# hucsmn/suffix_array

Hardware: AMD Instinct MI355X
Metric: input MB/s indexed (SA build) (higher is better)
Workload: dtype u8; 1 GPU; c3_english_256m: 268435456 bytes per GPU, seed base + rank, one independent text per GPU; n_bytes=268435456, sigma=57, symbols_per_key=13, refinement_rounds=9, text_rounds=0, radix_passes=25, unresolved_after_initial_sort=199000237

## Files before the change

suffix_array_amd/__init__.py:

```python
from __future__ import annotations

import ctypes
import os
from typing import Optional

import numpy as np

__all__ = ["MAX_LENGTH", "saca", "SuffixArray", "SuffixArrayError", "lib", "diag_lib", "library_path", "Stats", "last_host_timing",
           "saca_batch", "workspace_bytes", "device_pci_bus_id", "saca_device_ptr", "bucket_table", "check_integrity", "last_stats", "DeviceIndex", "pack", "unpack",
           "lcp", "saca_lcp", "last_lcp_stats", "lcp_work_bytes", "lcp_device_ptr", "LcpStats",
           "lcp_set_compare_cap", "last_search_stats", "SearchStats",
           "bwt", "unbwt", "bwt_device_ptr", "unbwt_device_ptr", "bwt_work_bytes", "unbwt_work_bytes", "last_unbwt_stats",
           "unbwt_set_walk_limits", "unbwt_set_splitter_spacing", "UnbwtStats",
           "repeat_lengths", "repeat_spans", "last_repeat_stats", "repeats_work_bytes", "repeat_spans_bound",
           "repeat_lengths_device_ptr", "repeat_spans_device_ptr", "RepeatStats", "REPEATS_ALL", "REPEATS_KEEP_FIRST",
           "lpf", "lz77", "lz77_decode", "lz77_literals", "last_lz_stats", "lz_work_bytes", "lpf_device_ptr", "lz77_device_ptr", "LzStats", "LZ_LITERAL",
           "repeated_substrings", "last_substr_stats", "substrings_work_bytes", "substrings_bound", "substrings_device_ptr", "SubstrQuery", "SubstrStats",
           "SUBSTR_ALL", "SUBSTR_BY_COUNT", "SUBSTR_BY_LENGTH", "SUBSTR_BY_COVER",
           "DocSubstrQuery", "DocSubstrStats", "SUBSTR_BY_DOCS", "last_doc_substr_stats", "doc_substrings_work_bytes",
           "MatchStats", "last_match_stats", "match_work_bytes", "match_set_group_cap", "match_set_group_lanes", "match_stats_device_ptr", "match_spans_device_ptr",
           "MATCH_NONE", "MATCH_TILE",
           "DocRepeatStats", "last_doc_repeat_stats", "doc_repeats_work_bytes", "DOCREP_ANY", "DOCREP_OTHER",
           "DocsStats", "last_docs_stats", "docs_set_chunk", "docs_work_bytes", "doc_of_device_ptr", "DOC_NONE", "DOC_SAMPLES",
           "DOC_CHUNK_MIN", "DOC_CHUNK_MAX", "DOC_CHUNK_DEFAULT",
# ... 532 lines not shown
        L.sa_amd_tok_index_next_tokens.argtypes = [c_vp, c_vp, c_vp, ctypes.c_int32, c_vp, c_vp, c_vp, c_vp, c_vp, c_vp, ctypes.c_int64, c_vp]
        L.sa_amd_tok_index_next_tokens.restype = ctypes.c_int32
        L.sa_amd_tok_index_infgram.argtypes = [c_vp, c_vp, c_vp, ctypes.c_int32, ctypes.c_int32, ctypes.c_int32, c_vp, c_vp, c_vp, c_vp, c_vp, c_vp,
                                               c_vp, ctypes.c_int64, c_vp]
        L.sa_amd_tok_index_infgram.restype = ctypes.c_int32
        L.sa_amd_last_tok_stats.argtypes = [c_vp]
        L.sa_amd_last_tok_stats.restype = None
        L.sa_amd_tok_index_infgram_score.argtypes = [c_vp, c_vp, ctypes.c_int64, c_vp, ctypes.c_int64, ctypes.c_int32, ctypes.c_int32, c_vp, c_vp,
                                                     c_vp, c_vp, c_vp, c_vp]
        L.sa_amd_tok_index_infgram_score.restype = ctypes.c_int32
        L.sa_amd_last_tok_score_stats.argtypes = [c_vp]
        L.sa_amd_last_tok_score_stats.restype = None
        for u16_name, u32_name in (("sa_amd_max_tokens_u16", "sa_amd_max_tokens_u32"), ("sa_amd_saca_u16", "sa_amd_saca_u32")) + tuple(
                ("sa_amd_tok_index_" + op, "sa_amd_tok32_index_" + op)
                for op in ("create", "destroy", "sa", "search", "next_tokens", "infgram", "infgram_score")):
            u16_fn, u32_fn = getattr(L, u16_name), getattr(L, u32_name)
            u32_fn.argtypes, u32_fn.restype = u16_fn.argtypes, u16_fn.restype
        _lib = L
    return _lib


_diag: Optional[ctypes.CDLL] = None


def diag_lib() -> ctypes.CDLL:
    global _diag
    if _diag is None:
        path = os.path.join(_HERE, "libsuffix_array_amd_diag.so")
        if not os.path.exists(path):
            raise ImportError(f"{path} not found: run __graft_entry__.build()")
        L = ctypes.CDLL(path)
        c_vp = ctypes.c_void_p
        L.sa_amd_test_sort_pairs.argtypes = [c_vp, c_vp, ctypes.c_int64, ctypes.c_int32, ctypes.c_int32]
        L.sa_amd_test_sort_pairs.restype = ctypes.c_int32
        L.sa_amd_test_sort_pairs32.argtypes = [c_vp, c_vp, ctypes.c_int64, ctypes.c_int32, ctypes.c_int32]
        L.sa_amd_test_sort_pairs32.restype = ctypes.c_int32
        L.sa_amd_test_sort_pairs_flags.argtypes = [c_vp, c_vp, ctypes.c_int64, ctypes.c_int32, ctypes.c_int32, c_vp, c_vp]
        L.sa_amd_test_sort_pairs_flags.restype = ctypes.c_int32
        L.sa_amd_debug_head_flags.argtypes = [ctypes.c_int32]
        L.sa_amd_debug_head_flags.restype = ctypes.c_int32
        L.sa_amd_debug_round_flags.argtypes = [ctypes.c_int32]
        L.sa_amd_debug_round_flags.restype = ctypes.c_int32
        L.sa_amd_debug_fill_blocks.argtypes = [ctypes.c_int32]
        L.sa_amd_debug_fill_blocks.restype = ctypes.c_int32
        L.sa_amd_last_stats.argtypes = [c_vp]
        L.sa_amd_test_sample_sort64.argtypes = [c_vp, c_vp, ctypes.c_int64, ctypes.c_int32, c_vp]
        L.sa_amd_test_sample_sort64.restype = ctypes.c_int32
        L.sa_amd_test_bucket_sort32.argtypes = [c_vp, c_vp, ctypes.c_int64, ctypes.c_int32, c_vp]
        L.sa_amd_test_bucket_sort32.restype = ctypes.c_int32
        L.sa_amd_test_lz_nsv.argtypes = [c_vp, ctypes.c_int64, c_vp, c_vp, c_vp]
        L.sa_amd_test_lz_nsv.restype = ctypes.c_int32
        L.sa_amd_test_build_keys.argtypes = [c_vp, ctypes.c_int32, c_vp, c_vp, c_vp]
        L.sa_amd_test_build_keys.restype = ctypes.c_int32
        L.sa_amd_debug_phase_cycles.argtypes = [c_vp, ctypes.c_int32]
        L.sa_amd_debug_phase_cycles.restype = ctypes.c_int32
        L.sa_amd_debug_group_sort_stamps.argtypes = [ctypes.c_int32]
        L.sa_amd_debug_group_sort_stamps.restype = ctypes.c_int32
        L.sa_amd_debug_rr_count_stamps.argtypes = [ctypes.c_int32]
        L.sa_amd_debug_rr_count_stamps.restype = ctypes.c_int32
        L.sa_amd_debug_sort_variant_count.restype = ctypes.c_int32
        L.sa_amd_debug_sort_variant_name.argtypes = [ctypes.c_int32]
        L.sa_amd_debug_sort_variant_name.restype = ctypes.c_char_p
        L.sa_amd_saca_u8.argtypes = [c_vp, c_vp, ctypes.c_int32]
        L.sa_amd_saca_u8.restype = ctypes.c_int32
        L.sa_amd_saca_device.argtypes = [c_vp, c_vp, ctypes.c_int32, c_vp, ctypes.c_int64, c_vp, c_vp]
        L.sa_amd_saca_device.restype = ctypes.c_int32
        L.sa_amd_workspace_bytes.argtypes = [ctypes.c_int32]
        L.sa_amd_workspace_bytes.restype = ctypes.c_int64
        L.sa_amd_version.restype = ctypes.c_char_p
        _diag = L
    return _diag


def device_pci_bus_id(device: int = 0) -> str:
    buf = ctypes.create_string_buffer(64)
    _check(lib().sa_amd_device_pci_bus_id(int(device), buf, 64))
    return buf.value.decode()


def _check(code: int) -> None:
    if code != 0:
        raise SuffixArrayError(code, lib().sa_amd_strerror(code).decode())


def _as_u8(s) -> np.ndarray:
    if isinstance(s, np.ndarray):
        if s.dtype != np.uint8 or not s.flags.c_contiguous:
            raise TypeError("text must be a contiguous uint8 array")
        return s
    return np.frombuffer(bytes(s), dtype=np.uint8) if len(s) else np.zeros(0, dtype=np.uint8)


def saca(s, sa: np.ndarray) -> None:
    t = _as_u8(s)
    assert t.size <= MAX_LENGTH
    assert t.size + 1 == sa.size
    if sa.dtype != np.uint32 or not sa.flags.c_contiguous or not sa.flags.writeable:
        raise TypeError("sa must be a writable contiguous uint32 array")
    _check(lib().sa_amd_saca_u8(t.ctypes.data, sa.ctypes.data, t.size))


def divsufsort(s, sa: np.ndarray) -> None:
    t = _as_u8(s)
    assert t.size == sa.size and sa.dtype == np.int32
    _check(lib().sa_amd_divsufsort(t.ctypes.data, sa.ctypes.data, t.size))

# ... 1219 lines not shown
```

suffix_array_amd/csrc/host/pipeline.hpp:

```cpp
#pragma once
#include "support.hpp"
#include "tuning.hpp"
#include "pool.hpp"
#include "sort.hpp"
#include "readback.hpp"

#include <functional>

namespace sa {

static inline Tuning env_tuning() { return Tuning::from_env(N_SORT_VARIANTS, N_SORT32_VARIANTS, N_OS_SHAPES64, N_OS_SHAPES32); }
static inline Tuning route_tuning()
{
    const Tuning tn = env_tuning();
    g_posted_off = tn.no_posted_readback;
    return tn;
}

constexpr size_t GRAM_MAX_ENTRIES = (size_t)1 << 24;
static_assert(GROUP_CAP_MAX == GS_CAP, "Tuning clamps SA_AMD_GROUP_CAP to the kernel's cap");

struct Workspace {
    uint64_t *keysA, *keysB, *keysC;
    uint32_t *valsA, *valsB, *isa, *U0, *U1, *G0, *G1;
// ... 101 lines not shown
static int scatter_binned(const SortScratch &ss, uint32_t *isa, uint32_t *pk, uint32_t *pv, uint32_t *altk, uint32_t *altv, int64_t count, int64_t n,
                          hipStream_t st, sa_amd_stats *local, const Tuning &tn, bool iota = false,
                          uint32_t *altk2 = nullptr, uint32_t *altv2 = nullptr)
{
    const int nb = bit_length((uint64_t)(n > 1 ? n : 1));
    int wlog = nb - 16;
    if (wlog < 10) wlog = 10;
    if (wlog > 15) wlog = 15;
    const bool two = nb > wlog && (tn.scatter_levels == 2 || (tn.scatter_levels == 0 && count >= ((int64_t)1 << 25)));
    SortResult<uint32_t> pr;
    if (two) {
        int rc;
        if (iota) {
            const int mid = wlog + RADIX_BITS < nb ? wlog + RADIX_BITS : nb;
            SortJob<uint32_t> first{ pk, nullptr, altk, altv, count, wlog, mid };
            first.iota = true;
            rc = sort_pairs32(first, ss, st, tn, &pr, local);
            if (rc) return rc;
            if (pr.passes != 1) return SA_AMD_EINTERNAL;
            if (mid < nb) {
                rc = sort_pairs32(SortJob<uint32_t>{ altk, altv, altk2, altv2, count, mid, nb }, ss, st, tn, &pr, local);
                if (rc) return rc;
            }
        } else {
            SortJob<uint32_t> both{ pk, pv, altk, altv, count, wlog, nb };
            both.keys_out2 = altk2;
            rc = sort_pairs32(both, ss, st, tn, &pr, local);
            if (rc) return rc;
        }
        const unsigned grid = (unsigned)ceil_div(count, SW_CHUNK);
        if (wlog <= 13)
            PROF(KC_SCATTER, count, st, hipLaunchKernelGGL((k_scatter_windows<13>), dim3(grid), dim3(SW_THREADS), 0, st, (const uint32_t *)pr.keys,
                                                           (const uint32_t *)pr.vals, isa, count, (uint32_t)n, wlog));
        else
            PROF(KC_SCATTER, count, st, hipLaunchKernelGGL((k_scatter_windows<15>), dim3(grid), dim3(SW_THREADS), 0, st, (const uint32_t *)pr.keys,
                                                           (const uint32_t *)pr.vals, isa, count, (uint32_t)n, wlog));
        return SA_AMD_OK;
    }
    const int shift = nb > RADIX_BITS ? nb - RADIX_BITS : 0;
    SortJob<uint32_t> one{ pk, pv, altk, altv, count, shift, shift + RADIX_BITS };
    one.iota = iota;
    const int rc = sort_pairs32(one, ss, st, tn, &pr, local);
    if (rc) return rc;
    PROF(KC_SCATTER, count, st, hipLaunchKernelGGL((k_scatter_pairs<uint32_t>), dim3((unsigned)ceil_div(count, 1024)), dim3(256), 0, st,
                                                   (const uint32_t *)pr.keys, (const uint32_t *)pr.vals, isa, count, (uint32_t)n));
    return SA_AMD_OK;
}

}
#include "refine_round.hpp"
namespace sa {

static int choose_gram_keys(const uint8_t *dT, int64_t n, KeyParams *Pp, int *key_bits, const Workspace &w, hipStream_t st,
                            const Tuning &tn, bool trace)
{
    KeyParams &P = *Pp;
    const uint64_t se = P.sigma;
    const uint64_t cap = (uint64_t)((size_t)n < GRAM_MAX_ENTRIES ? (size_t)n : GRAM_MAX_ENTRIES);
    int g = 0;
    uint64_t S = 1;
    for (int t = 1; t <= 8; ++t) {
        if (S * se > cap) break;
        S *= se; g = t;
        if (tn.gram_g >= 2 && g == tn.gram_g) break;
    }
    if (g < 2) return SA_AMD_OK;
    uint64_t top = 1;
    for (int t = 0; t + 1 < g; ++t) top *= se;
    const int64_t gtiles = ceil_div((int64_t)S, GT_TILE);
    HIP_TRY(hipMemsetAsync(w.gram_flags, 0, (size_t)S, st));
    PROF(KC_MISC, n, st, hipLaunchKernelGGL((k_gram_mark), dim3((unsigned)ceil_div(ceil_div(n, KB_TILE), GM_TPW)), dim3(KB_THREADS), 0, st, dT, n, P, g,
                                            (uint32_t)top, w.gram_flags));
    PROF(KC_MISC, (int64_t)S, st, hipLaunchKernelGGL((k_gram_count), dim3((unsigned)gtiles), dim3(GT_THREADS), 0, st,
                                            (const uint8_t *)w.gram_flags, (int64_t)S, w.tcnt));
    PROF(KC_RR_SCAN, gtiles, st, hipLaunchKernelGGL((k_rr_scan), dim3(1), dim3(SPINE_THREADS), 0, st, w.tcnt, w.thead, gtiles, w.total));
    uint32_t D = 0;
    { const int rcw = read_words(&D, w.total, 4, st); if (rcw) return rcw; }
    int m = 0;
    unsigned __int128 pw = 1;
    while (D >= 2 && (m + 1) * g <= 64 && pw * D <= ((unsigned __int128)1 << 64)) { pw *= D; ++m; }
    int tail = 0;
    while (m > 0 && tail < tn.gram_tail_max && m * g + tail + 1 <= 64 && pw * se <= ((unsigned __int128)1 << 64)) { pw *= se; ++tail; }
    const int gram_bits = m > 0 ? bit_length((uint64_t)(pw - 1)) : 0;
    const int plain_passes = (int)ceil_div(*key_bits, RADIX_BITS), gram_passes = (int)ceil_div(gram_bits, RADIX_BITS);
    const int syms = m * g + tail;
    const bool better = m > 0 && (syms > P.k || (syms == P.k && gram_passes < plain_passes));
    if (trace) fprintf(stderr, "suffix_array_amd: gram keys: %u of %llu %d-grams occur -> %d symbols (%d grams + %d plain) in %d bits (plain: %d in %d) -> %s\n",
                       D, (unsigned long long)S, g, syms, m, tail, gram_bits, P.k, *key_bits, better ? "gram keys" : "plain keys");
    if (!better) return SA_AMD_OK;
    PROF(KC_MISC, (int64_t)S, st, hipLaunchKernelGGL((k_gram_table), dim3((unsigned)gtiles), dim3(GT_THREADS), 0, st,
                                            (const uint8_t *)w.gram_flags, (int64_t)S, (const uint32_t *)w.tcnt, w.gram_table));
    P.gram = g; P.gram_m = m; P.gram_tail = tail; P.gram_top = (uint32_t)top; P.gram_D = D; P.gram_table = w.gram_table;
    P.bits = 0; P.k = syms; P.mask = ~0ull;
    *key_bits = gram_bits;
    return SA_AMD_OK;
}

struct EarlyDownload {
    int off = 0;
    int64_t threshold = 0;
    std::function<void(hipEvent_t)> start;
    std::function<int64_t()> stop;
    bool started = false;
    int64_t m_snap = 0;
    int64_t covered = 0;
    int64_t holes = 0;
    const uint32_t *d_bits = nullptr, *d_tile_off = nullptr, *d_holes = nullptr;
    hipEvent_t ev = nullptr;
};

struct DeviceBuild : BuildCore {
    EarlyDownload *early = nullptr;
    bool trace = false;
    double trace_t = 0;
    double lap() { const double t = now_ms(), d = t - trace_t; trace_t = t; return d; }
    bool timing_only() const
    {
#ifdef SA_AMD_DIAG
        return tn.timing_only_initial_sort;
#else
        return false;
#endif
    }
    KeyParams P, Ptext;
    int sigma = 0, key_bits = 0, top_shift = 0;
    bool force_dense = false, text_ok = false, probe_dense = false;
    SortResult<uint64_t> sr;
    const uint32_t *sorted32 = nullptr;
    int bucket_top_bits = 0;
    bool flat_text = false;
    bool bucket_finished = false;
    uint64_t *sorted0 = nullptr;
    int64_t tiles = 0, depth = 0;
    uint32_t m32 = 0;
    bool lists_ready = false, finished32 = false, fused64 = false, sparse = false;
    bool isa_tail_ranks = false;
    bool tnext_scanned = false;
    int s_sym = 0, tkb = 0;
    bool unary_done = false;
// ... 43 lines not shown
    int choose_bucket_bits() const
    {
        if (tn.no_bucket_sort || n < tn.bucket_min_n || n <= 1) return 0;
        const bool wide_ok = onesweep_on(w.ss, tn) && tn.onesweep32_shape == 0;
        if (tn.bucket_bits == 18 && wide_ok) return 18;
        if (tn.bucket_bits == 16) return 16;
        const bool value_bits = wide_ok && !tn.no_value_bits && !tn.no_text_keys && g_bits <= 30 &&
                                ((sigma == 256 && P.bits == 8) || (sigma == 4 && P.bits == 2 && !tn.no_packed_text));
        if (value_bits && (n >> 16) > 7500 && (n >> 18) * 10 <= bucket_cap_max() * 9) return 18;
        if ((n >> 16) * 10 <= bucket_cap(2) * 9) return 16;
        if (wide_ok && (n >> 18) * 10 <= bucket_cap_max() * 9) return 18;
        if ((n >> 16) * 10 <= bucket_cap_max() * 9) return 16;
        return 0;
    }

    bool flat_rule_applies() const { return n >= 2 && n < tn.top32_probe_min_n && n < ((int64_t)1 << 24) && !tn.no_flat_rule; }

    template <int ISA_MODE>
    int rr_apply_setup(const RrApply &a)
    {
        const uint64_t *k = sr.keys;
        if (head_flags)
            return isa_tail_ranks ? rr_apply<true, false, ISA_MODE, uint64_t, true, true>(k, a) : rr_apply<true, false, ISA_MODE, uint64_t, false, true>(k, a);
        return isa_tail_ranks ? rr_apply<true, false, ISA_MODE, uint64_t, true>(k, a) : rr_apply<true, false, ISA_MODE>(k, a);
    }
    int rebuild_sorted_keys()
    {
        if (!head_flags) return SA_AMD_OK;
        int64_t blocks = ceil_div(n, GK_THREADS);
        if (blocks > 65536) blocks = 65536;
        PROF(KC_GATHER, n, st, hipLaunchKernelGGL((k_keys_of_suffixes), dim3((unsigned)blocks), dim3(GK_THREADS), 0, st, dT, P, n, (const uint32_t *)SA, sr.keys));
        head_flags = nullptr;
        if (trace) fprintf(stderr, "suffix_array_amd: sorted keys rebuilt from the suffix array (the route taken reads them)\n");
        return SA_AMD_OK;
    }
    RrApply first_args(uint32_t n_text, uint32_t *has_isa = nullptr) const
    {
        RrApply a;
        a.V = SA; a.m = n; a.SA = SA; a.ISA = w.isa; a.Uo = L.U; a.Go = L.G; a.Vo = L.V; a.n_text = n_text; a.has_isa = has_isa;
        return a;
    }
    int count_sample_dups(int64_t S, size_t zero_bytes)
    {
        const uint32_t H = (uint32_t)S * 4u;
        HIP_TRY(hipMemsetAsync(w.keysB, 0xff, (size_t)H * 8, st));
        HIP_TRY(hipMemsetAsync(w.total, 0, zero_bytes, st));
        PROF(KC_MISC, S, st, hipLaunchKernelGGL((k_count_sample_dups), dim3((unsigned)(ceil_div(S, 256) < 4096 ? ceil_div(S, 256) : 4096)), dim3(256), 0, st, (const uint64_t *)w.keysA, S,
                                                (unsigned long long *)w.keysB, H - 1u, w.total));
        return SA_AMD_OK;
    }
    int build_keys64(uint32_t *vals0, uint8_t *packed_out, const FirstCounts &fc, bool counted)
    {
        const int nb0 = key_bits < RADIX_BITS ? key_bits : RADIX_BITS;
        const unsigned grid = (unsigned)ceil_div(ceil_div(n, KB_TILE), KB_TPW);
        PROF(KC_BUILD_KEYS, n, st, hipLaunchKernelGGL((P.gram > 0 ? k_build_keys<false, true> : k_build_keys<false>), dim3(grid), dim3(KB_THREADS), 0, st, dT, n, P, w.keysA, vals0,
                                                      (uint32_t *)nullptr, 0, packed_out, counted ? fc.counts : (uint32_t *)nullptr, fc.chunk_elems, fc.G, (1u << nb0) - 1u, 0));
        return SA_AMD_OK;
    }
    int zero_finish_records()
    {
        HIP_TRY(hipMemsetAsync(w.surv_bits, 0, ((size_t)n + 31) / 32 * 4, st));
        HIP_TRY(hipMemsetAsync(w.tcnt, 0, (size_t)ceil_div(n, RR_TILE) * 4, st));
        HIP_TRY(hipMemsetAsync(w.thead, 0, (size_t)ceil_div(n, RR_TILE) * 4, st));
        HIP_TRY(hipMemsetAsync(w.total, 0, 16, st));
        HIP_TRY(hipMemsetAsync(w.chg, 0, (size_t)RR_CHG_COUNTERS * 32 * 4, st));
        return SA_AMD_OK;
    }

    int geometry_and_probes()
    {
        int rc;
        HIP_TRY(hipMemsetAsync(w.hist, 0, 256 * 4, st));
        {
            int64_t blocks = ceil_div(ceil_div(n, 16), BH_THREADS);
            if (blocks > 2048) blocks = 2048;
            if (blocks < 1) blocks = 1;
            const bool counts = flat_rule_applies();
            if (counts) PROF(KC_BYTE_HIST, n, st, hipLaunchKernelGGL((k_byte_hist_counts), dim3((unsigned)(blocks > 256 ? 256 : blocks)), dim3(BH_THREADS), 0, st, dT, n, w.hist));
            else PROF(KC_BYTE_HIST, n, st, hipLaunchKernelGGL((k_byte_hist), dim3((unsigned)blocks), dim3(BH_THREADS), 0, st, dT, n, w.hist));
        }
        uint32_t hist[256];
        { const int rcw = read_words(hist, w.hist, sizeof(hist), st); if (rcw) return rcw; }
        int kb_max = tn.key_bits_max;
        if (flat_rule_applies()) {
            double h0 = 0.0; int used = 0;
            for (int c = 0; c < 256; ++c)
                if (hist[c]) { const double pc = (double)hist[c] / (double)n; h0 -= pc * std::log2(pc); ++used; }
            if (used >= 2 && h0 > std::log2((double)used) - 0.01) {
                int kb = (bit_length((uint64_t)(n - 1)) + 20 + 7) / 8 * 8;
                if (kb < 32) kb = 32;
                if (kb < kb_max) kb_max = kb;
                flat_text = true;
            }
        }
        key_bits = make_key_params(hist, &P, &sigma, kb_max);
        local.sigma = sigma; local.bits_per_symbol = P.bits; local.symbols_per_key = P.k;
        if (sigma == 1 && !tn.no_unary_shortcut) {
            int64_t blocks = ceil_div(n, 256 * 16);
            if (blocks > 16384) blocks = 16384;
            PROF(KC_MISC, n, st, hipLaunchKernelGGL((k_fill_descending), dim3((unsigned)blocks), dim3(256), 0, st, SA, n));
            unary_done = true;
            return SA_AMD_OK;
        }

        g_bits = bit_length((uint64_t)(n - 1 > 0 ? n - 1 : 1));
        bucket_top_bits = choose_bucket_bits();
        force_dense = tn.force_dense;
// ... 569 lines not shown
```

suffix_array_amd/csrc/kernels/keys.hpp:

```cpp
#pragma once
#include "common.hpp"

namespace sa {

constexpr int BH_THREADS = 256;

__global__ __launch_bounds__(BH_THREADS) void k_byte_hist(const uint8_t *__restrict__ T, int64_t n,
                                                           uint32_t *__restrict__ hist)
{
    __shared__ uint32_t h[256];
    h[threadIdx.x] = 0;
    __syncthreads();
    const uintptr_t addr = (uintptr_t)T;
    int64_t head = (int64_t)((16 - (addr & 15)) & 15);
    if (head > n) head = n;
    const int64_t nvec = (n - head) / 16;
    const uint4 *V = (const uint4 *)(T + head);
    const int64_t gtid = (int64_t)blockIdx.x * BH_THREADS + threadIdx.x;
    const int64_t gstride = (int64_t)gridDim.x * BH_THREADS;
    for (int64_t i = gtid; i < nvec; i += gstride) {
        uint4 q = V[i];
        uint32_t w4[4] = { q.x, q.y, q.z, q.w };
#pragma unroll
        for (int a = 0; a < 4; ++a) {
// ... 21 lines not shown
    const int64_t nvec = (n - head) / 16;
    const uint4 *V = (const uint4 *)(T + head);
    const int64_t gtid = (int64_t)blockIdx.x * BH_THREADS + threadIdx.x;
    const int64_t gstride = (int64_t)gridDim.x * BH_THREADS;
    for (int64_t i = gtid; i < nvec; i += gstride) {
        const uint4 q = V[i];
        const uint32_t w4[4] = { q.x, q.y, q.z, q.w };
#pragma unroll
        for (int a = 0; a < 4; ++a) {
#pragma unroll
            for (int b = 0; b < 4; ++b) atomicAdd(&mine[(w4[a] >> (8 * b)) & 255u], 1u);
        }
    }
    if (blockIdx.x == 0) {
        for (int64_t i = threadIdx.x; i < head; i += BH_THREADS) atomicAdd(&mine[T[i]], 1u);
        for (int64_t i = head + nvec * 16 + threadIdx.x; i < n; i += BH_THREADS) atomicAdd(&mine[T[i]], 1u);
    }
    __syncthreads();
    uint32_t c = 0;
#pragma unroll
    for (int w = 0; w < BH_THREADS / WAVE; ++w) c += h[w][threadIdx.x];
    if (c) atomicAdd(&hist[threadIdx.x], c);
}

constexpr int KB_THREADS = 256;
constexpr int KB_ITEMS = 8;
constexpr int KB_TILE = KB_THREADS * KB_ITEMS;
constexpr int KB_HALO = 64 + 8;

struct KeyParams {
    uint8_t code[256];
    int32_t bits;
    int32_t k;
    uint64_t mask;
    uint64_t sigma;
    uint64_t top;
    const uint8_t *packed;
    int32_t gram, gram_m, gram_tail;
    uint32_t gram_top;
    uint64_t gram_D;
    const uint4 *gram_table;
};

__device__ __forceinline__ uint32_t gram_rank(const uint4 *__restrict__ table, uint32_t idx)
{
    const uint4 rec = table[idx >> 6];
    const uint64_t bits = ((uint64_t)rec.y << 32) | rec.x;
    return rec.z + (uint32_t)__popcll(bits & ((1ull << (idx & 63u)) - 1ull));
}

__device__ __forceinline__ void kb_stage_codes(const uint8_t *__restrict__ T, int64_t n, int64_t base, const uint8_t *lcode, uint8_t *c, int tid);

constexpr int KB_TPW = 8;
constexpr int GM_LOG = 13;
constexpr int GRAM_CACHE = 1 << GM_LOG;
constexpr int GM_TPW = 64;
__device__ __forceinline__ uint32_t gram_slot(uint32_t idx) { return (idx * 2654435761u) >> (32 - GM_LOG); }

template <bool TOP32, bool GRAM = false>
__global__ __launch_bounds__(KB_THREADS) void k_build_keys(const uint8_t *__restrict__ T, int64_t n,
                                                            KeyParams P, uint64_t *__restrict__ keys,
                                                            uint32_t *__restrict__ vals, uint32_t *__restrict__ keys32,
                                                            int top_shift, uint8_t *__restrict__ packed_out,
                                                            uint32_t *__restrict__ counts, int64_t chunk_elems, int G, uint32_t dmask, int dshift = 0)
{
    __shared__ uint8_t lcode[256];
    __shared__ __attribute__((aligned(16))) uint8_t c[KB_TILE + KB_HALO];
    __shared__ uint32_t dhist[512];
    __shared__ uint32_t gc[GRAM ? KB_TILE + KB_HALO : 1];
    const int tid = threadIdx.x;
    lcode[tid] = P.code[tid];
    for (int d = tid; d < 512; d += KB_THREADS) dhist[d] = 0;

    __syncthreads();
    const int64_t tiles = (n + KB_TILE - 1) / KB_TILE;
    const int64_t tile0 = (int64_t)blockIdx.x * KB_TPW;
    const int64_t tile1 = tile0 + KB_TPW < tiles ? tile0 + KB_TPW : tiles;
  for (int64_t tile = tile0; tile < tile1; ++tile) {
    const int64_t base = tile * KB_TILE;
    kb_stage_codes(T, n, base, lcode, c, tid);
    __syncthreads();
    const int p0 = tid * KB_ITEMS;
    const int k = P.k, bits = P.bits;
    uint64_t kk[KB_ITEMS];
    if (GRAM) {
        const int g = P.gram, m = P.gram_m;
        const uint32_t sg = (uint32_t)P.sigma;
        for (int o = tid; o + g <= KB_TILE + KB_HALO; o += KB_THREADS) {
            uint32_t idx = 0;
            for (int t = 0; t < g; ++t) idx = idx * sg + (uint32_t)c[o + t];
            gc[o] = gram_rank(P.gram_table, idx);
        }
        __syncthreads();
        const uint64_t D = P.gram_D;
        const int tail = P.gram_tail;
#pragma unroll
        for (int r = 0; r < KB_ITEMS; ++r) {
            uint64_t key = 0;
            for (int j = 0; j < m; ++j) key = key * D + (uint64_t)gc[p0 + r + g * j];
            for (int t = 0; t < tail; ++t) key = key * (uint64_t)sg + (uint64_t)c[p0 + r + g * m + t];
            kk[r] = key;
        }
    } else if (bits > 0) {
        const uint64_t mask = P.mask;
        uint64_t key = 0;
        for (int j = 0; j < k; ++j) key = (key << bits) | (uint64_t)c[p0 + j];
        kk[0] = key;
#pragma unroll
        for (int r = 1; r < KB_ITEMS; ++r) {
            key = ((key << bits) | (uint64_t)c[p0 + k - 1 + r]) & mask;
            kk[r] = key;
        }
    } else {
        const uint64_t sigma = P.sigma, top = P.top;
        uint64_t key = 0;
        for (int j = 0; j < k; ++j) key = key * sigma + (uint64_t)c[p0 + j];
        kk[0] = key;
#pragma unroll
        for (int r = 1; r < KB_ITEMS; ++r) {
            key = (key - (uint64_t)c[p0 + r - 1] * top) * sigma + (uint64_t)c[p0 + k - 1 + r];
            kk[r] = key;
        }
    }
    const int64_t g0 = base + p0;
    if (packed_out && g0 < n) {
        uint32_t val = 0;
#pragma unroll
        for (int r = 0; r < KB_ITEMS; ++r) val = (val << bits) | (uint32_t)c[p0 + r];
        uint8_t *po = packed_out + (g0 >> 3) * bits;
        for (int b = 0; b < bits; ++b) po[b] = (uint8_t)(val >> (8 * (bits - 1 - b)));
    }
    if (g0 + KB_ITEMS <= n) {
        if (TOP32) {
            uint4 *ko = (uint4 *)(keys32 + g0);
            ko[0] = make_uint4((uint32_t)(kk[0] >> top_shift), (uint32_t)(kk[1] >> top_shift), (uint32_t)(kk[2] >> top_shift),
                               (uint32_t)(kk[3] >> top_shift));
            ko[1] = make_uint4((uint32_t)(kk[4] >> top_shift), (uint32_t)(kk[5] >> top_shift), (uint32_t)(kk[6] >> top_shift),
                               (uint32_t)(kk[7] >> top_shift));
        } else {
            ulonglong2 *ko = (ulonglong2 *)(keys + g0);
#pragma unroll
            for (int r = 0; r < KB_ITEMS / 2; ++r) ko[r] = make_ulonglong2(kk[2 * r], kk[2 * r + 1]);
        }
        if (vals) {
            uint4 *vo = (uint4 *)(vals + g0);
            const uint32_t v0 = (uint32_t)g0;
            vo[0] = make_uint4(v0, v0 + 1, v0 + 2, v0 + 3);
            vo[1] = make_uint4(v0 + 4, v0 + 5, v0 + 6, v0 + 7);
        }
    } else {
#pragma unroll
        for (int r = 0; r < KB_ITEMS; ++r)
            if (g0 + r < n) {
                if (TOP32) keys32[g0 + r] = (uint32_t)(kk[r] >> top_shift); else keys[g0 + r] = kk[r];
// ... 267 lines not shown
```

suffix_array_amd/csrc/sa_diag.h:

```cpp
#ifndef SUFFIX_ARRAY_AMD_DIAG_H
#define SUFFIX_ARRAY_AMD_DIAG_H
#include "../../include/suffix_array_amd.h"
#ifdef __cplusplus
extern "C" {
#endif
int32_t sa_amd_debug_phase_cycles(uint64_t *out, int32_t count);
int32_t sa_amd_debug_group_sort_stamps(int32_t on);
int32_t sa_amd_debug_rr_count_stamps(int32_t on);
int32_t sa_amd_debug_rerank_routes(int32_t flags);
int32_t sa_amd_debug_head_flags(int32_t mode);
int32_t sa_amd_debug_round_flags(int32_t mode);
int32_t sa_amd_debug_doc_tf_bounds(int32_t mode);
int32_t sa_amd_debug_dsub_plain_atomics(int32_t mode);
int32_t sa_amd_debug_fill_blocks(int32_t pattern);
int32_t sa_amd_debug_sort_variant_count(void);
const char *sa_amd_debug_sort_variant_name(int32_t index);
int32_t sa_amd_test_sort_pairs(uint64_t *keys, uint32_t *vals, int64_t count, int32_t begin_bit, int32_t end_bit);
int32_t sa_amd_test_sort_pairs_flags(const uint64_t *keys, uint32_t *vals, int64_t count, int32_t begin_bit, int32_t end_bit,
                                     uint8_t *flags_out, uint64_t *keys_out);
int32_t sa_amd_test_sample_sort64(uint64_t *keys, uint32_t *vals, int64_t count, int32_t key_bits, int32_t *done);
int32_t sa_amd_test_sort_pairs32(uint32_t *keys, uint32_t *vals, int64_t count, int32_t begin_bit, int32_t end_bit);
int32_t sa_amd_test_lz_nsv(const uint32_t *dA, int64_t n, uint32_t *dPsv, uint32_t *dNsv, int64_t *counters);
int32_t sa_amd_test_bucket_sort32(uint32_t *keys, uint32_t *vals, int64_t count, int32_t top_bits, uint32_t *largest);
int32_t sa_amd_test_build_keys(const uint8_t *T, int32_t n, uint64_t *keys, int32_t *bits, int32_t *k);
int32_t sa_amd_proto_induce_l(const uint8_t *T, const uint8_t *typeL, uint32_t *SA, int32_t n, const uint32_t *head,
                              double *ms, uint64_t *counters);
#ifdef __cplusplus
}
#endif
#endif
```

suffix_array_amd/csrc/sa_diag.inc:

```

SA_EXPORT int32_t sa_amd_debug_phase_cycles(uint64_t *out, int32_t count)
{
    unsigned long long h[16] = { 0 };
    if (hipMemcpyFromSymbol(h, HIP_SYMBOL(sa::g_phase_cycles), sizeof(h)) != hipSuccess) return SA_AMD_EHIP;
    for (int i = 0; i < count && i < 16; ++i) out[i] = h[i];
    unsigned long long z[16] = { 0 };
    (void)hipMemcpyToSymbol(HIP_SYMBOL(sa::g_phase_cycles), z, sizeof(z));
    return 16;
}

SA_EXPORT int32_t sa_amd_debug_group_sort_stamps(int32_t on)
{
    const int v = on ? 1 : 0;
    return hipMemcpyToSymbol(HIP_SYMBOL(sa::g_gs_stamp_on), &v, sizeof(v)) == hipSuccess ? SA_AMD_OK : SA_AMD_EHIP;
}

SA_EXPORT int32_t sa_amd_debug_rr_count_stamps(int32_t on)
{
    const int v = on ? 1 : 0;
    return hipMemcpyToSymbol(HIP_SYMBOL(sa::g_rr_stamp_on), &v, sizeof(v)) == hipSuccess ? SA_AMD_OK : SA_AMD_EHIP;
}

SA_EXPORT int32_t sa_amd_debug_rerank_routes(int32_t flags)
{
// ... 201 lines not shown
        const FirstCounts fc = sort_first_counts(ss, tn, count, true);
        HIP_TRY(hipMemset(fc.zero_ptr, 0, fc.zero_bytes));
        hipLaunchKernelGGL(k_test_count_digit, dim3(256), dim3(256), 0, nullptr, (const uint32_t *)k, count, 32 - top_bits, 511u, fc.counts, fc.chunk_elems, fc.G);
        HIP_TRY(hipGetLastError());
        counted = true;
    }
    SortJob<uint32_t> job{ k, v, k + N, v + N, count, 32 - top_bits, 32 };
    job.first_counted = counted; job.rbits = rbits;
    rc = sort_pairs32(job, ss, nullptr, tn, &sr);
    if (rc != SA_AMD_OK) return rc;
    uint32_t *kout = sr.keys == k ? k + N : k, *vout = v + 2 * N;
    bool done = false;
    rc = bucket_sort32(sr.keys, sr.vals, kout, vout, count, top_bits, dbs.as<uint32_t>(), ss.err + 2, nullptr, tn, &done, largest);
    if (rc != SA_AMD_OK) return rc;
    HIP_TRY(hipDeviceSynchronize());
    { uint32_t e[4] = { 0, 0, 0, 0 }; HIP_TRY(hipMemcpy(e, ss.err, 16, hipMemcpyDeviceToHost)); if (e[0] || e[3]) return SA_AMD_EINTERNAL; }
    if (!done) return 1;
    HIP_TRY(hipMemcpy(keys, kout, (size_t)count * 4, hipMemcpyDeviceToHost));
    HIP_TRY(hipMemcpy(vals, vout, (size_t)count * 4, hipMemcpyDeviceToHost));
    return SA_AMD_OK;
}

SA_EXPORT int32_t sa_amd_test_build_keys(const uint8_t *T, int32_t n, uint64_t *keys, int32_t *bits, int32_t *k)
{
    using namespace sa;
    if (n <= 0 || !T || !keys) return SA_AMD_EINVAL;
    if (sa::device_count() <= 0) return SA_AMD_ENODEVICE;
    DevBuf dT, dk, dv, dh;
    int32_t rc;
    if ((rc = dT.alloc((size_t)n))) return rc;
    if ((rc = dk.alloc((size_t)n * 8))) return rc;
    if ((rc = dv.alloc((size_t)n * 4))) return rc;
    if ((rc = dh.alloc(1024))) return rc;
    HIP_TRY(hipMemcpy(dT.p, T, (size_t)n, hipMemcpyHostToDevice));
    HIP_TRY(hipMemset(dh.p, 0, 1024));
    int64_t blocks = ceil_div(ceil_div((int64_t)n, 16), BH_THREADS);
    if (blocks > 2048) blocks = 2048;
    if (blocks < 1) blocks = 1;
    hipLaunchKernelGGL(k_byte_hist, dim3((unsigned)blocks), dim3(BH_THREADS), 0, nullptr, dT.as<const uint8_t>(), (int64_t)n, dh.as<uint32_t>());
    uint32_t hist[256];
    HIP_TRY(hipMemcpy(hist, dh.p, 1024, hipMemcpyDeviceToHost));
    KeyParams P; int sigma;
    make_key_params(hist, &P, &sigma);
    hipLaunchKernelGGL((k_build_keys<false>), dim3((unsigned)ceil_div(ceil_div((int64_t)n, KB_TILE), KB_TPW)), dim3(KB_THREADS), 0, nullptr, dT.as<const uint8_t>(),
                       (int64_t)n, P, dk.as<uint64_t>(), dv.as<uint32_t>(), (uint32_t *)nullptr, 0, (uint8_t *)nullptr,
                       (uint32_t *)nullptr, (int64_t)KB_TILE, 1, 0u);
    HIP_TRY(hipGetLastError());
    HIP_TRY(hipDeviceSynchronize());
    HIP_TRY(hipMemcpy(keys, dk.p, (size_t)n * 8, hipMemcpyDeviceToHost));
    if (bits) *bits = P.bits;
    if (k) *k = P.k;
    return SA_AMD_OK;
}

SA_EXPORT int32_t sa_amd_proto_induce_l(const uint8_t *T, const uint8_t *typeL, uint32_t *SA, int32_t n, const uint32_t *head,
                                        double *ms, uint64_t *counters)
{
    using namespace sa;
    if (n <= 0 || !T || !typeL || !SA || !head || !ms || !counters) return SA_AMD_EINVAL;
    if (sa::device_count() <= 0) return SA_AMD_ENODEVICE;
    const size_t N = (size_t)n;
    DevBuf dT, dL, dS, dH, dC;
    int32_t rc;
    if ((rc = dT.alloc(N))) return rc;
    if ((rc = dL.alloc(N / 8 + 8))) return rc;
    if ((rc = dS.alloc((N + 1) * 4))) return rc;
    if ((rc = dH.alloc(1024))) return rc;
    if ((rc = dC.alloc(16))) return rc;
    HIP_TRY(hipMemcpy(dT.p, T, N, hipMemcpyHostToDevice));
    HIP_TRY(hipMemcpy(dL.p, typeL, N / 8 + 1, hipMemcpyHostToDevice));
    HIP_TRY(hipMemcpy(dS.p, SA, (N + 1) * 4, hipMemcpyHostToDevice));
    HIP_TRY(hipMemcpy(dH.p, head, 1024, hipMemcpyHostToDevice));
    HIP_TRY(hipMemset(dC.p, 0, 16));
    hipEvent_t a, b;
    HIP_TRY(hipEventCreate(&a)); HIP_TRY(hipEventCreate(&b));
    HIP_TRY(hipEventRecord(a, nullptr));
    hipLaunchKernelGGL(k_induce_l_sweep, dim3(1), dim3(64), 0, nullptr, dT.as<const uint8_t>(), dL.as<const uint8_t>(), dS.as<uint32_t>(),
                       (int64_t)n, dH.as<const uint32_t>(), dC.as<unsigned long long>());
    HIP_TRY(hipGetLastError());
    HIP_TRY(hipEventRecord(b, nullptr));
    HIP_TRY(hipEventSynchronize(b));
    float t = 0.f;
    HIP_TRY(hipEventElapsedTime(&t, a, b));
    (void)hipEventDestroy(a); (void)hipEventDestroy(b);
    *ms = t;
    HIP_TRY(hipMemcpy(SA, dS.p, (N + 1) * 4, hipMemcpyDeviceToHost));
    HIP_TRY(hipMemcpy(counters, dC.p, 16, hipMemcpyDeviceToHost));
    return SA_AMD_OK;
}

SA_EXPORT int32_t sa_amd_test_lz_nsv(const uint32_t *dA, int64_t n, uint32_t *dPsv, uint32_t *dNsv, int64_t *counters)
{
    using namespace sa;
    if (n <= 0 || n > 0x7fffffffLL || !dA || !dPsv || !dNsv || !counters) return SA_AMD_EINVAL;
    if (sa::device_count() <= 0) return SA_AMD_ENODEVICE;
    DevBuf dl, dc;
    int32_t rc;
    if ((rc = dl.alloc(((size_t)n / 31 + 64) * 4))) return rc;
    if ((rc = dc.alloc(256))) return rc;
    HIP_TRY(hipMemset(dc.p, 0, 256));
    rc = lz_nsv(dA, n, dPsv, dNsv, dl.as<uint32_t>(), nullptr, nullptr, dc.as<unsigned long long>(), nullptr);
    if (rc != SA_AMD_OK) return rc;
    HIP_TRY(hipDeviceSynchronize());
    unsigned long long cw[LZ_C_WORDS];
    HIP_TRY(hipMemcpy(cw, dc.p, sizeof(cw), hipMemcpyDeviceToHost));
    counters[0] = (int64_t)cw[LZ_C_UNRES];
// ... 6 lines not shown
```

Measured before the change: 6072 MB/s.

## Cache gram ranks in shared memory and compute rolling gram indices per thread

The gram-key build kernel now computes each thread's gram indices with a rolling update from two 8-byte register words, instead of a per-position loop over shared memory. Rank lookups go through a per-block hashed shared-memory cache of (index, rank) pairs, so repeated grams skip the global bitmap-table popcount lookup. Gram-branch blocks now handle 16 tiles each instead of 8, which spreads the cache initialisation over more work. The per-block cache adds shared-memory pressure and may lower occupancy. Test hooks and a force flag for choosing gram keys are also added.

Measured after the change: 6164 MB/s, median of 6. +1.5%, better.

```diff
diff --git a/suffix_array_amd/__init__.py b/suffix_array_amd/__init__.py
--- a/suffix_array_amd/__init__.py
+++ b/suffix_array_amd/__init__.py
@@ -608,6 +608,12 @@
         L.sa_amd_test_lz_nsv.restype = ctypes.c_int32
         L.sa_amd_test_build_keys.argtypes = [c_vp, ctypes.c_int32, c_vp, c_vp, c_vp]
         L.sa_amd_test_build_keys.restype = ctypes.c_int32
+        L.sa_amd_test_gram_keys.argtypes = [c_vp, ctypes.c_int32, ctypes.c_int32, ctypes.c_int32, c_vp, c_vp, c_vp, c_vp]
+        L.sa_amd_test_gram_keys.restype = ctypes.c_int32
+        L.sa_amd_test_gram_front_params.argtypes = [c_vp, ctypes.c_int32]
+        L.sa_amd_test_gram_front_params.restype = ctypes.c_int32
+        L.sa_amd_test_gram_slot.argtypes = [ctypes.c_uint32, ctypes.c_int32]
+        L.sa_amd_test_gram_slot.restype = ctypes.c_uint32
         L.sa_amd_debug_phase_cycles.argtypes = [c_vp, ctypes.c_int32]
         L.sa_amd_debug_phase_cycles.restype = ctypes.c_int32
         L.sa_amd_debug_group_sort_stamps.argtypes = [ctypes.c_int32]
diff --git a/suffix_array_amd/csrc/host/pipeline.hpp b/suffix_array_amd/csrc/host/pipeline.hpp
--- a/suffix_array_amd/csrc/host/pipeline.hpp
+++ b/suffix_array_amd/csrc/host/pipeline.hpp
@@ -177,7 +177,7 @@
 namespace sa {
 
 static int choose_gram_keys(const uint8_t *dT, int64_t n, KeyParams *Pp, int *key_bits, const Workspace &w, hipStream_t st,
-                            const Tuning &tn, bool trace)
+                            const Tuning &tn, bool trace, bool force = false)
 {
     KeyParams &P = *Pp;
     const uint64_t se = P.sigma;
@@ -209,7 +209,7 @@
     const int gram_bits = m > 0 ? bit_length((uint64_t)(pw - 1)) : 0;
     const int plain_passes = (int)ceil_div(*key_bits, RADIX_BITS), gram_passes = (int)ceil_div(gram_bits, RADIX_BITS);
     const int syms = m * g + tail;
-    const bool better = m > 0 && (syms > P.k || (syms == P.k && gram_passes < plain_passes));
+    const bool better = m > 0 && (force || syms > P.k || (syms == P.k && gram_passes < plain_passes));
     if (trace) fprintf(stderr, "suffix_array_amd: gram keys: %u of %llu %d-grams occur -> %d symbols (%d grams + %d plain) in %d bits (plain: %d in %d) -> %s\n",
                        D, (unsigned long long)S, g, syms, m, tail, gram_bits, P.k, *key_bits, better ? "gram keys" : "plain keys");
     if (!better) return SA_AMD_OK;
@@ -359,7 +359,7 @@
     int build_keys64(uint32_t *vals0, uint8_t *packed_out, const FirstCounts &fc, bool counted)
     {
         const int nb0 = key_bits < RADIX_BITS ? key_bits : RADIX_BITS;
-        const unsigned grid = (unsigned)ceil_div(ceil_div(n, KB_TILE), KB_TPW);
+        const unsigned grid = (unsigned)ceil_div(ceil_div(n, KB_TILE), P.gram > 0 ? KB_GRAM_TPW : KB_TPW);
         PROF(KC_BUILD_KEYS, n, st, hipLaunchKernelGGL((P.gram > 0 ? k_build_keys<false, true> : k_build_keys<false>), dim3(grid), dim3(KB_THREADS), 0, st, dT, n, P, w.keysA, vals0,
                                                       (uint32_t *)nullptr, 0, packed_out, counted ? fc.counts : (uint32_t *)nullptr, fc.chunk_elems, fc.G, (1u << nb0) - 1u, 0));
         return SA_AMD_OK;
diff --git a/suffix_array_amd/csrc/kernels/keys.hpp b/suffix_array_amd/csrc/kernels/keys.hpp
--- a/suffix_array_amd/csrc/kernels/keys.hpp
+++ b/suffix_array_amd/csrc/kernels/keys.hpp
@@ -97,10 +97,14 @@
 __device__ __forceinline__ void kb_stage_codes(const uint8_t *__restrict__ T, int64_t n, int64_t base, const uint8_t *lcode, uint8_t *c, int tid);
 
 constexpr int KB_TPW = 8;
+constexpr int KB_GRAM_TPW = 16;
+constexpr int KR_LOG = 11;
+constexpr int RANK_CACHE = 1 << KR_LOG;
 constexpr int GM_LOG = 13;
 constexpr int GRAM_CACHE = 1 << GM_LOG;
 constexpr int GM_TPW = 64;
-__device__ __forceinline__ uint32_t gram_slot(uint32_t idx) { return (idx * 2654435761u) >> (32 - GM_LOG); }
+__host__ __device__ __forceinline__ uint32_t gram_slot(uint32_t idx) { return (idx * 2654435761u) >> (32 - GM_LOG); }
+__host__ __device__ __forceinline__ uint32_t rank_slot(uint32_t idx) { return (idx * 2654435761u) >> (32 - KR_LOG); }
 
 template <bool TOP32, bool GRAM = false>
 __global__ __launch_bounds__(KB_THREADS) void k_build_keys(const uint8_t *__restrict__ T, int64_t n,
@@ -112,15 +116,17 @@
     __shared__ uint8_t lcode[256];
     __shared__ __attribute__((aligned(16))) uint8_t c[KB_TILE + KB_HALO];
     __shared__ uint32_t dhist[512];
-    __shared__ uint32_t gc[GRAM ? KB_TILE + KB_HALO : 1];
+    __shared__ __attribute__((aligned(16))) uint32_t gc[GRAM ? KB_TILE + KB_HALO : 1];
+    __shared__ unsigned long long s_rank[GRAM ? RANK_CACHE : 1];
+    constexpr int TPW = GRAM ? KB_GRAM_TPW : KB_TPW;
     const int tid = threadIdx.x;
     lcode[tid] = P.code[tid];
     for (int d = tid; d < 512; d += KB_THREADS) dhist[d] = 0;
-
+    if (GRAM) for (int i = tid; i < RANK_CACHE; i += KB_THREADS) s_rank[i] = ~0ull;
     __syncthreads();
     const int64_t tiles = (n + KB_TILE - 1) / KB_TILE;
-    const int64_t tile0 = (int64_t)blockIdx.x * KB_TPW;
-    const int64_t tile1 = tile0 + KB_TPW < tiles ? tile0 + KB_TPW : tiles;
+    const int64_t tile0 = (int64_t)blockIdx.x * TPW;
+    const int64_t tile1 = tile0 + TPW < tiles ? tile0 + TPW : tiles;
   for (int64_t tile = tile0; tile < tile1; ++tile) {
     const int64_t base = tile * KB_TILE;
     kb_stage_codes(T, n, base, lcode, c, tid);
@@ -130,21 +136,70 @@
     uint64_t kk[KB_ITEMS];
     if (GRAM) {
         const int g = P.gram, m = P.gram_m;
-        const uint32_t sg = (uint32_t)P.sigma;
-        for (int o = tid; o + g <= KB_TILE + KB_HALO; o += KB_THREADS) {
+        const uint32_t sg = (uint32_t)P.sigma, gtop = P.gram_top;
+        const int extra = g * (m - 1);
+        constexpr int NI = KB_ITEMS + 1;
+        const uint2 q0 = *(const uint2 *)(c + p0), q1 = *(const uint2 *)(c + p0 + 8);
+        const uint64_t w0 = ((uint64_t)q0.y << 32) | q0.x, w1 = ((uint64_t)q1.y << 32) | q1.x;
+        const uint64_t wn = g == 8 ? w1 : (w0 >> (8 * g)) | (w1 << (64 - 8 * g));
+        uint32_t ix[NI];
+        {
             uint32_t idx = 0;
-            for (int t = 0; t < g; ++t) idx = idx * sg + (uint32_t)c[o + t];
-            gc[o] = gram_rank(P.gram_table, idx);
-        }
+            for (int t = 0; t < g; ++t) idx = idx * sg + (uint32_t)((w0 >> (8 * t)) & 255u);
+#pragma unroll
+            for (int r = 0; r < KB_ITEMS; ++r) {
+                ix[r] = idx;
+                idx = (idx - (uint32_t)((w0 >> (8 * r)) & 255u) * gtop) * sg + (uint32_t)((wn >> (8 * r)) & 255u);
+            }
+            idx = 0;
+            if (tid < extra) for (int t = 0; t < g; ++t) idx = idx * sg + (uint32_t)c[KB_TILE + tid + t];
+            ix[KB_ITEMS] = idx;
+        }
+        unsigned long long e[NI];
+        bool miss[NI];
+#pragma unroll
+        for (int r = 0; r < NI; ++r) {
+            e[r] = __hip_atomic_load(&s_rank[rank_slot(ix[r])], __ATOMIC_RELAXED, __HIP_MEMORY_SCOPE_WORKGROUP);
+            miss[r] = (r < KB_ITEMS || tid < extra) && (uint32_t)(e[r] >> 32) != ix[r];
+        }
+        uint4 rec[NI];
+#pragma unroll
+        for (int r = 0; r < NI; ++r) rec[r] = miss[r] ? P.gram_table[ix[r] >> 6] : make_uint4(0u, 0u, 0u, 0u);
+        uint32_t rk[NI];
+#pragma unroll
+        for (int r = 0; r < NI; ++r) {
+            rk[r] = (uint32_t)e[r];
+            if (miss[r]) {
+                const uint64_t bits = ((uint64_t)rec[r].y << 32) | rec[r].x;
+                rk[r] = rec[r].z + (uint32_t)__popcll(bits & ((1ull << (ix[r] & 63u)) - 1ull));
+                __hip_atomic_store(&s_rank[rank_slot(ix[r])], ((unsigned long long)ix[r] << 32) | rk[r], __ATOMIC_RELAXED,
+                                   __HIP_MEMORY_SCOPE_WORKGROUP);
+            }
+        }
+        *(uint4 *)(gc + p0) = make_uint4(rk[0], rk[1], rk[2], rk[3]);
+        *(uint4 *)(gc + p0 + 4) = make_uint4(rk[4], rk[5], rk[6], rk[7]);
+        if (tid < extra) gc[KB_TILE + tid] = rk[KB_ITEMS];
         __syncthreads();
         const uint64_t D = P.gram_D;
         const int tail = P.gram_tail;
 #pragma unroll
-        for (int r = 0; r < KB_ITEMS; ++r) {
-            uint64_t key = 0;
-            for (int j = 0; j < m; ++j) key = key * D + (uint64_t)gc[p0 + r + g * j];
-            for (int t = 0; t < tail; ++t) key = key * (uint64_t)sg + (uint64_t)c[p0 + r + g * m + t];
-            kk[r] = key;
+        for (int r = 0; r < KB_ITEMS; ++r) kk[r] = (uint64_t)rk[r];
+        for (int j = 1; j < m; ++j) {
+            const uint32_t *q = gc + p0 + g * j;
+            uint32_t v[KB_ITEMS];
+            if (((g * j) & 3) == 0) {
+                const uint4 a = *(const uint4 *)q, b = *(const uint4 *)(q + 4);
+                v[0] = a.x; v[1] = a.y; v[2] = a.z; v[3] = a.w; v[4] = b.x; v[5] = b.y; v[6] = b.z; v[7] = b.w;
+            } else {
+#pragma unroll
+                for (int r = 0; r < KB_ITEMS; ++r) v[r] = q[r];
+            }
+#pragma unroll
+            for (int r = 0; r < KB_ITEMS; ++r) kk[r] = kk[r] * D + (uint64_t)v[r];
+        }
+        for (int t = 0; t < tail; ++t) {
+#pragma unroll
+            for (int r = 0; r < KB_ITEMS; ++r) kk[r] = kk[r] * (uint64_t)sg + (uint64_t)c[p0 + r + g * m + t];
         }
     } else if (bits > 0) {
         const uint64_t mask = P.mask;
diff --git a/suffix_array_amd/csrc/sa_diag.h b/suffix_array_amd/csrc/sa_diag.h
--- a/suffix_array_amd/csrc/sa_diag.h
+++ b/suffix_array_amd/csrc/sa_diag.h
@@ -23,6 +23,10 @@
 int32_t sa_amd_test_lz_nsv(const uint32_t *dA, int64_t n, uint32_t *dPsv, uint32_t *dNsv, int64_t *counters);
 int32_t sa_amd_test_bucket_sort32(uint32_t *keys, uint32_t *vals, int64_t count, int32_t top_bits, uint32_t *largest);
 int32_t sa_amd_test_build_keys(const uint8_t *T, int32_t n, uint64_t *keys, int32_t *bits, int32_t *k);
+int32_t sa_amd_test_gram_keys(const uint8_t *T, int32_t n, int32_t g, int32_t tail_max, uint64_t *keys_out, uint32_t *D_out,
+                              int32_t *bits_out, int32_t *k_out);
+int32_t sa_amd_test_gram_front_params(int32_t *out, int32_t count);
+uint32_t sa_amd_test_gram_slot(uint32_t idx, int32_t which);
 int32_t sa_amd_proto_induce_l(const uint8_t *T, const uint8_t *typeL, uint32_t *SA, int32_t n, const uint32_t *head,
                               double *ms, uint64_t *counters);
 #ifdef __cplusplus
diff --git a/suffix_array_amd/csrc/sa_diag.inc b/suffix_array_amd/csrc/sa_diag.inc
--- a/suffix_array_amd/csrc/sa_diag.inc
+++ b/suffix_array_amd/csrc/sa_diag.inc
@@ -277,6 +277,53 @@
     if (k) *k = P.k;
     return SA_AMD_OK;
 }
+
+SA_EXPORT int32_t sa_amd_test_gram_keys(const uint8_t *T, int32_t n, int32_t g, int32_t tail_max, uint64_t *keys_out, uint32_t *D_out,
+                                        int32_t *bits_out, int32_t *k_out)
+{
+    using namespace sa;
+    if (n <= 0 || !T || !keys_out || g < 0 || g > 8 || tail_max < 0 || tail_max > 8) return SA_AMD_EINVAL;
+    if (sa::device_count() <= 0) return SA_AMD_ENODEVICE;
+    Tuning tn = env_tuning();
+    tn.gram_g = g; tn.gram_tail_max = tail_max;
+    DevBuf dT, dk, dw;
+    int32_t rc;
+    if ((rc = dT.alloc((size_t)n))) return rc;
+    if ((rc = dk.alloc((size_t)n * 8))) return rc;
+    if ((rc = dw.alloc(carve(nullptr, n).bytes))) return rc;
+    const Workspace w = carve(dw.p, n);
+    HIP_TRY(hipMemcpy(dT.p, T, (size_t)n, hipMemcpyHostToDevice));
+    HIP_TRY(hipMemset(w.hist, 0, 1024));
+    int64_t blocks = ceil_div(ceil_div((int64_t)n, 16), BH_THREADS);
+    if (blocks > 2048) blocks = 2048;
+    hipLaunchKernelGGL(k_byte_hist, dim3((unsigned)blocks), dim3(BH_THREADS), 0, nullptr, dT.as<const uint8_t>(), (int64_t)n, w.hist);
+    uint32_t hist[256];
+    HIP_TRY(hipMemcpy(hist, w.hist, 1024, hipMemcpyDeviceToHost));
+    KeyParams P; int sigma, key_bits;
+    key_bits = make_key_params(hist, &P, &sigma);
+    if ((rc = choose_gram_keys(dT.as<const uint8_t>(), (int64_t)n, &P, &key_bits, w, nullptr, tn, false, true))) return rc;
+    if (P.gram == 0) return 1;
+    hipLaunchKernelGGL((k_build_keys<false, true>), dim3((unsigned)ceil_div(ceil_div((int64_t)n, KB_TILE), KB_GRAM_TPW)), dim3(KB_THREADS), 0, nullptr,
+                       dT.as<const uint8_t>(), (int64_t)n, P, dk.as<uint64_t>(), (uint32_t *)nullptr, (uint32_t *)nullptr, 0, (uint8_t *)nullptr,
+                       (uint32_t *)nullptr, (int64_t)KB_TILE, 1, 0u);
+    HIP_TRY(hipGetLastError());
+    HIP_TRY(hipDeviceSynchronize());
+    HIP_TRY(hipMemcpy(keys_out, dk.p, (size_t)n * 8, hipMemcpyDeviceToHost));
+    if (D_out) *D_out = (uint32_t)P.gram_D;
+    if (bits_out) *bits_out = key_bits;
+    if (k_out) *k_out = P.k;
+    return SA_AMD_OK;
+}
+
+SA_EXPORT int32_t sa_amd_test_gram_front_params(int32_t *out, int32_t count)
+{
+    const int32_t v[5] = { sa::KR_LOG, sa::KB_GRAM_TPW, sa::GM_LOG, sa::GM_TPW, sa::KB_TILE };
+    int32_t i = 0;
+    for (; out && i < count && i < 5; ++i) out[i] = v[i];
+    return i;
+}
+
+SA_EXPORT uint32_t sa_amd_test_gram_slot(uint32_t idx, int32_t which) { return which ? sa::gram_slot(idx) : sa::rank_slot(idx); }
 
 SA_EXPORT int32_t sa_amd_proto_induce_l(const uint8_t *T, const uint8_t *typeL, uint32_t *SA, int32_t n, const uint32_t *head,
                                         double *ms, uint64_t *counters)
```
